# lfilipozzi/PathPlanning

Measured on AMD Instinct MI355X. Metric: hybrid_astar_plans_per_sec_1024x1024, higher is better.
Workload: dtype f64

## Files before the change

__graft_entry__.py:

```python
import os
import subprocess
import sys

os.environ.setdefault("GPU_MAX_HW_QUEUES", "2")

ROOT = os.path.dirname(os.path.abspath(__file__))
if ROOT not in sys.path:
    sys.path.insert(0, ROOT)


def build():
    from pathplanning_amd import build as b
    lib = b.build(force=False)
    assert os.path.exists(lib), lib
    b.build_pyplanning()
    b.build_plugin_test()
    b.build_pipeline_footprint_test()
    b.build_pipeline_postprocess_test()
    b.build_row_test()
    subprocess.check_call(["make", "-C", os.path.join(ROOT, "oracle"), os.path.join(ROOT, "oracle", "libppo.so")])
    if os.path.isdir("/root/reference/planner/src"):
        subprocess.check_call(["make", "-C", os.path.join(ROOT, "oracle"), "ref"])
    subprocess.check_call([sys.executable, "-c", "import ctypes, sys; ctypes.CDLL(sys.argv[1])", lib])
    import pathplanning_amd
    print("built", lib)


def smoke():
    sys.path.insert(0, os.path.join(ROOT, "tests"))
    import numpy as np
    import pathplanning_amd as pa
    import torch
    assert torch.cuda.is_available(), "smoke() needs a GPU"
    import oracle_lib as O
# ... 72 lines not shown
```

pathplanning_amd/build.py:

```python
import os
import subprocess
import sys

HERE = os.path.dirname(os.path.abspath(__file__))
CSRC = os.path.join(HERE, "csrc")
LIB_DIR = os.path.join(HERE, "lib")
LIB = os.path.join(LIB_DIR, "libpphip.so")
SOURCES = ["pp_capi.hip", "pp_kernels_basic.hip", "pp_paths.hip", "pp_footprint.hip", "pp_gvd.hip", "pp_wavefront.hip", "pp_wavefront_tiles.hip", "pp_planner.hip", "pp_rrt.hip", "pp_grid_astar.hip"]
HEADERS = sorted(f for f in os.listdir(CSRC) if f.endswith(".hpp")) + [os.path.join("..", "..", "include", "pp_hip.h")]
FLAGS = ["--offload-arch=gfx950", "-O3", "-std=c++17", "-ffp-contract=off", "-fPIC", "-shared"]


def hipcc():
    for c in (os.environ.get("HIPCC"), "/opt/rocm/bin/hipcc", "hipcc"):
        if c and (os.path.isabs(c) and os.path.exists(c) or not os.path.isabs(c)):
            return c
    return "hipcc"


def stale():
    if not os.path.exists(LIB):
        return True
    t = os.path.getmtime(LIB)
    deps = [os.path.join(CSRC, s) for s in SOURCES + HEADERS]
# ... 63 lines not shown
    return out


def build_row_test(verbose=True):
    out = os.path.join(LIB_DIR, "test_row_primitives")
    src = os.path.join(HERE, "..", "tests", "cpp", "test_row_primitives.hip")
    if os.path.exists(out) and os.path.getmtime(out) > max(os.path.getmtime(src), os.path.getmtime(os.path.join(CSRC, "pp_row_primitives.hpp"))):
        return out
    cmd = [hipcc(), "--offload-arch=gfx950", "-O2", "-I", CSRC, "-I", os.path.join(HERE, "..", "include"), src, "-o", out]
    if verbose:
        print(" ".join(cmd), file=sys.stderr)
    subprocess.check_call(cmd)
    return out


if __name__ == "__main__":
    build(force="--force" in sys.argv)
    print(LIB)
    print(build_pyplanning())
    print(build_plugin_test())
    print(build_pipeline_footprint_test())
    print(build_pipeline_postprocess_test())
    print(build_row_test())
```

pathplanning_amd/csrc/pp_capi.hip:

```cpp
#include "pp_internal.hpp"

#include <cmath>
#include <cstdio>
#include <cstring>
#include <memory>

namespace pph {

static thread_local std::string g_lastError;

void set_error(const std::string& msg) { g_lastError = msg; }
int hip_fail(hipError_t e, const char* what)
{
	g_lastError = std::string(what) + ": " + hipGetErrorString(e);
	return e == hipErrorNoDevice ? PP_ERR_NO_DEVICE : PP_ERR_HIP;
}

}

using namespace pph;

ppd::MapView pp_map::view() const
{
	ppd::MapView v;
// ... 445 lines not shown
		return PP_ERR_INVALID;
	}
	if (!map->pathcost) {
		set_error("path-cost grid not uploaded (pp_map_upload_path_cost)");
		return PP_ERR_INVALID;
	}
	rp.arcLength = params->spatial_resolution * 1.5;
	rp.spatialRes = params->spatial_resolution;
	rp.angularRes = params->angular_resolution;
	rp.lat.set(params->spatial_resolution, params->angular_resolution);
	rp.forwardMult = params->forward_cost_multiplier;
	rp.reverseMult = params->reverse_cost_multiplier;
	rp.voronoiMult = params->voronoi_cost_multiplier;
	rp.voroDiagRes = (float)(map->desc.resolution * std::sqrt(2.0));
	rp.headingAlias = params->heading_alias;
	pt.n = n_primitives;
	for (int i = 0; i < n_primitives; i++) {
		pt.kappa[i] = curvature_host[i];
		pt.invKappa[i] = curvature_host[i] != 0.0 ? 1 / curvature_host[i] : 0.0;
		pt.backward[i] = direction_host[i] == 1;
	}
	return PP_OK;
}

int pp_rollout_children_dev(pp_map* map, const pp_hybrid_params* params, int32_t n_primitives, const double* curvature_host, const int32_t* direction_host,
	int64_t n_parents, const double* parents_dev, uint8_t* valid_dev, double* pose_dev, int32_t* key_dev, double* cost_dev, double* length_dev)
{
	if (int rc = check_map(map, true))
		return rc;
	RolloutParams rp;
// ... 467 lines not shown
```

pathplanning_amd/csrc/pp_device.hpp:

```cpp
#pragma once

#include <hip/hip_runtime.h>
#include <stdint.h>

namespace ppd {

#define PPD_INLINE __device__ __forceinline__

constexpr double kPi = 3.14159265358979323846;

#ifndef PP_FIELD_TILE_LOG2
#define PP_FIELD_TILE_LOG2 3
#endif
constexpr int kFieldTileLog2 = PP_FIELD_TILE_LOG2, kFieldTile = 1 << kFieldTileLog2, kFieldTileMask = kFieldTile - 1;
__host__ __device__ inline size_t field_tiled_index(int cols, int row, int col)
{
	const int tpr = (cols + kFieldTileMask) >> kFieldTileLog2;
	return ((size_t)((row >> kFieldTileLog2) * tpr + (col >> kFieldTileLog2)) << (2 * kFieldTileLog2)) | (size_t)(((row & kFieldTileMask) << kFieldTileLog2) | (col & kFieldTileMask));
}
__host__ __device__ inline size_t field_tiled_elems(int rows, int cols)
{
	return (size_t)((rows + kFieldTileMask) >> kFieldTileLog2) * (size_t)((cols + kFieldTileMask) >> kFieldTileLog2) * (size_t)(kFieldTile * kFieldTile);
}
constexpr double kPi2 = 1.57079632679489661923;
// ... 131 lines not shown
		lt = wrap_theta(theta);
	const double qx = div_by(x - m.gx, (double)m.res, m.invRes), qy = div_by(y - m.gy, (double)m.res, m.invRes);
	const bool inRange = qx > -2147483649.0 && qx < 2147483648.0 && qy > -2147483649.0 && qy < 2147483648.0;
	const int row = (int)qx, col = (int)qy;
	const bool bounds = !(lx < m.lbx) & !(lx > m.ubx) & !(ly < m.lby) & !(ly > m.uby) & !(lt < m.lbt) & !(lt > m.ubt);
	const bool inside = inRange & ((unsigned)row < (unsigned)m.rows) & ((unsigned)col < (unsigned)m.cols);
#ifdef PP_CS_EXPERIMENT_NO_GATHER
	const uint32_t cell = inside ? (uint32_t)(row & 1) : 0u;
#else
	const uint32_t cell = inside ? (uint32_t)row * (uint32_t)m.cols + (uint32_t)col : 0u;
#endif
	const uint32_t bit = (validBits[cell >> 5] >> (cell & 31)) & 1u;
	return bounds & inside & (bit != 0u);
}

PPD_INLINE Pose constant_steer(const Pose& from, double kappa, double dist)
{
	Pose to = from;
	if (fabs(kappa) > 1e-9) {
		to.t += dist * kappa;
		to.x += 1 / kappa * (sin(to.t) - sin(from.t));
		to.y += 1 / kappa * (-cos(to.t) + cos(from.t));
	} else {
		to.x += dist * cos(from.t);
		to.y += dist * sin(from.t);
	}
	return to;
}

struct Arc {
// ... 31 lines not shown
			to.t += d * kappa;
			sincos(to.t, &s, &c);
			to.x += invKappa * (s - sinF);
			to.y += invKappa * (-c + cosF);
		} else {
			to.x += d * cosF;
			to.y += d * sinF;
		}
		return to;
	}
	PPD_INLINE Pose interpolate(double ratio) const
	{
		double s, c;
		return interpolate_sc(ratio, s, c);
	}
};

struct Segment {
	double x0, y0, x1, y1;
	double length;
	PPD_INLINE Pose interpolate(double ratio) const
	{
		Pose p;
		p.x = (1 - ratio) * x0 + ratio * x1;
		p.y = (1 - ratio) * y0 + ratio * y1;
		p.t = 0.0;
		return p;
	}
};

PPD_INLINE float fmin4(double a, double b, double c, double d)
// ... 29 lines not shown
		checks++;
		if (!is_state_valid(m, s.x, s.y, s.t, distance)) {
			last = (float)(lastValidLength / pathLength);
			return false;
		}
		lastValidLength = length;
		float distToMapBorder = fmin4(s.x - m.lbx, m.ubx - s.x, s.y - m.lby, m.uby - s.y);
		float deltaLength = distance - m.minSafeRadius;
		deltaLength = fminf(deltaLength, distToMapBorder);
		length += (double)fmaxf(deltaLength, m.minInterp);
	}
	last = 1.0f;
	return true;
}

template <typename PathT>
PPD_INLINE bool is_path_valid_from(const MapView& m, const PathT& path, const Pose& init, float firstDist, float& last, int& checks)
{
	const double pathLength = path.length;
	if (pathLength == 0.0) {
		last = 1.0f;
		checks++;
		return !(firstDist < 0.0f);
	}
	checks++;
	if (firstDist < 0.0f) {
		last = 0.0f;
		return false;
	}
	float distance = firstDist;
	double lastValidLength = 0.0;
	double length = 0.0;
	{
		const float distToMapBorder = fmin4(init.x - m.lbx, m.ubx - init.x, init.y - m.lby, m.uby - init.y);
		float deltaLength = distance - m.minSafeRadius;
		deltaLength = fminf(deltaLength, distToMapBorder);
		length += (double)fmaxf(deltaLength, m.minInterp);
	}
	while (length < pathLength) {
		if (checks > (1 << 22)) {
			last = (float)(lastValidLength / pathLength);
			return false;
		}
		Pose s = path.interpolate(length / pathLength);
		checks++;
		if (!is_state_valid(m, s.x, s.y, s.t, distance)) {
			last = (float)(lastValidLength / pathLength);
			return false;
		}
		lastValidLength = length;
		float distToMapBorder = fmin4(s.x - m.lbx, m.ubx - s.x, s.y - m.lby, m.uby - s.y);
		float deltaLength = distance - m.minSafeRadius;
		deltaLength = fminf(deltaLength, distToMapBorder);
		length += (double)fmaxf(deltaLength, m.minInterp);
	}
	last = 1.0f;
	return true;
}

template <typename PathT>
PPD_INLINE double voronoi_cost(const MapView& m, const PathT& path, float interpLength, double voronoiCostMultiplier)
{
	float voronoiCost = 0.0f;
	const double pathLength = path.length;
	if (0.0 < pathLength) {
		double lastLength = 0.0;
		if (interpLength > 0.0f)
			for (double length = 0.0; length < pathLength; length += (double)interpLength) {
				if (length == lastLength && length != 0.0)
					break;
				lastLength = length;
			}
		Pose p = path.interpolate(lastLength / pathLength);
		int row, col;
		world_to_cell(m, p.x, p.y, row, col);
		row = min(max(row, 0), m.rows - 1);
		col = min(max(col, 0), m.cols - 1);
		voronoiCost = m.pathcost[(size_t)row * m.cols + col];
	}
	voronoiCost *= interpLength;
	return voronoiCostMultiplier * (double)voronoiCost;
}

template <typename PathT>
PPD_INLINE void voronoi_cost_issue(const MapView& m, const PathT& path, float interpLength, float& raw)
{
	raw = 0.0f;
	const double pathLength = path.length;
	if (0.0 < pathLength) {
		double lastLength = 0.0;
		if (interpLength > 0.0f)
			for (double length = 0.0; length < pathLength; length += (double)interpLength) {
				if (length == lastLength && length != 0.0)
					break;
				lastLength = length;
			}
		Pose p = path.interpolate(lastLength / pathLength);
		int row, col;
		world_to_cell(m, p.x, p.y, row, col);
		row = min(max(row, 0), m.rows - 1);
		col = min(max(col, 0), m.cols - 1);
		raw = m.pathcost[(size_t)row * m.cols + col];
	}
}
PPD_INLINE double voronoi_cost_finish(float raw, float interpLength, double voronoiCostMultiplier)
{
	float voronoiCost = raw;
	voronoiCost *= interpLength;
	return voronoiCostMultiplier * (double)voronoiCost;
}

PPD_INLINE int alias_heading_bin(int theta)
{
	int t = theta;
	while ((double)t > kPi)
		t = (int)((double)t - 2 * kPi);
	while ((double)t < -kPi)
		t = (int)((double)t + 2 * kPi);
// ... 20 lines not shown
```

pathplanning_amd/csrc/pp_footprint_device.hpp:

```cpp
#pragma once

#include "pp_device.hpp"

namespace ppd {

constexpr int kFootprintMaxDiscs = 8;

struct Footprint {
	int n;
	int anyOffset;
	double rho;
	double ox[kFootprintMaxDiscs], oy[kFootprintMaxDiscs];
	float r[kFootprintMaxDiscs];
	int slot[kFootprintMaxDiscs];
};

PPD_INLINE void disc_centre(const Footprint& fp, int i, double x, double y, double s, double c, double& cx, double& cy)
{
	if (fp.ox[i] == 0.0 && fp.oy[i] == 0.0) {
		cx = x;
		cy = y;
	} else {
		cx = (x + fp.ox[i] * c) - fp.oy[i] * s;
		cy = (y + fp.ox[i] * s) + fp.oy[i] * c;
// ... 154 lines not shown
	last = 1.0f;
	return true;
}

PPD_INLINE float fp_border_sc(const MapView& m, const Footprint& fp, double x, double y, double s, double c)
{
	double b = dmin4(x - m.lbx, m.ubx - x, y - m.lby, m.uby - y, __builtin_huge_val());
	for (int i = 0; i < fp.n; i++) {
		double cx, cy;
		disc_centre(fp, i, x, y, s, c, cx, cy);
		b = dmin4(b, cx - m.lbx, m.ubx - cx, cy - m.lby, m.uby - cy);
	}
	return (float)b;
}

PPD_INLINE bool is_arc_valid_fp_from(const MapView& m, const Footprint& fp, float gain, const ArcSC& path, float firstClearance, float& last, int& checks)
{
	const double pathLength = path.length;
	if (pathLength == 0.0) {
		last = 1.0f;
		checks++;
		return !(firstClearance < 0.0f);
	}
	checks++;
	if (firstClearance < 0.0f) {
		last = 0.0f;
		return false;
	}
	double lastValidLength = 0.0;
	double length = 0.0;
	{
		const float border = fp_border_sc(m, fp, path.init.x, path.init.y, path.sinF, path.cosF);
		const float deltaLength = fminf(firstClearance, border) / gain;
		length += (double)fmaxf(deltaLength, m.minInterp);
	}
	while (length < pathLength) {
		if (checks > (1 << 22)) {
			last = (float)(lastValidLength / pathLength);
			return false;
		}
		double s, c;
		const Pose p = path.interpolate_sc(length / pathLength, s, c);
		checks++;
		float clearance, border;
		if (!fp_state_valid_sc(m, fp, p.x, p.y, p.t, s, c, clearance, border)) {
			last = (float)(lastValidLength / pathLength);
			return false;
		}
		lastValidLength = length;
		const float deltaLength = fminf(clearance, border) / gain;
		length += (double)fmaxf(deltaLength, m.minInterp);
	}
	last = 1.0f;
	return true;
}

}
```

pathplanning_amd/csrc/pp_internal.hpp:

```cpp
#pragma once

#include <hip/hip_runtime.h>
#include <stdint.h>
#include <string>
#include <vector>

#include "../../include/pp_hip.h"
#include "pp_device.hpp"
#include "pp_footprint_device.hpp"

namespace pph {

void set_error(const std::string& msg);
int hip_fail(hipError_t e, const char* what);

#define PP_HIP_TRY(expr)                       \
	do {                                       \
		hipError_t _e = (expr);                \
		if (_e != hipSuccess)                  \
			return pph::hip_fail(_e, #expr);   \
	} while (0)

template <typename H, hipError_t (*Release)(H)>
class Owner {
// ... 51 lines not shown
constexpr int kMaxPrimitives = 128;
struct PrimTable {
	int n;
	double kappa[kMaxPrimitives];
	double invKappa[kMaxPrimitives];
	int8_t backward[kMaxPrimitives];
};

struct RolloutParams {
	double arcLength;
	double spatialRes, angularRes;
	ppd::Resolutions lat;
	double forwardMult, reverseMult, voronoiMult;
	float voroDiagRes;
	int headingAlias;
};

struct NonHoloDesc {
	int nx, ny, na;
	double spatialRes, angularRes, offX, offY;
	double rmin;
	float reverseCost, forwardCost, switchCost;
	double minMult;
	int negativeKRead;
};

hipError_t launch_d2_to_distance(hipStream_t s, const int32_t* d2, float* dist, int64_t n, float res);
hipError_t launch_occ_to_u8(hipStream_t s, const int32_t* occ, uint8_t* occ8, int64_t n);
hipError_t launch_check_states(hipStream_t s, const ppd::MapView& m, int64_t n, const double* poses, uint8_t* valid);
hipError_t launch_check_states_fused(hipStream_t s, const ppd::MapView& m, int64_t n, uint64_t seed, uint64_t* count);
// ... 147 lines not shown
```

pathplanning_amd/csrc/pp_kernels_basic.hip:

```cpp
#include "pp_internal.hpp"

#include <mutex>

#include <cstdlib>
#include "pp_rs_device.hpp"

using namespace ppd;

namespace {

constexpr int kBlock = 256;

inline int grid_for(int64_t n, int block, int maxBlocks = 256 * 16)
{
	int64_t b = (n + block - 1) / block;
	if (b < 1)
		b = 1;
	if (b > maxBlocks)
		b = maxBlocks;
	return (int)b;
}

__global__ void k_d2_to_distance(const int32_t* __restrict__ d2, float* __restrict__ dist, int64_t n, float res)
{
// ... 227 lines not shown
		discretize_pose(child, rp.lat, rp.headingAlias, ix, iy, it);
		float lastValidRatio;
		int checks = 0;
		bool ok = true;
		if (!is_path_valid(m, a, a.init, lastValidRatio, checks)) {
			child = a.interpolate((double)lastValidRatio);
			a.length *= (double)lastValidRatio;
			discretize_pose(child, rp.lat, rp.headingAlias, ix, iy, it);
			if (ix == pix && iy == piy && it == pit)
				ok = false;
		}
		double c = 0.0;
		if (ok) {
			double pathCost = (a.backward ? rp.reverseMult : rp.forwardMult) * a.length;
			double switchingCost = 0.0;
			double voro = voronoi_cost(m, a, rp.voroDiagRes, rp.voronoiMult);
			c = pathCost + switchingCost + voro;
		}
		valid[idx] = ok ? 1 : 0;
		pose[3 * idx] = child.x;
		pose[3 * idx + 1] = child.y;
		pose[3 * idx + 2] = child.t;
		key[3 * idx] = ix;
		key[3 * idx + 1] = iy;
		key[3 * idx + 2] = it;
		cost[idx] = c;
		lengthOut[idx] = ok ? a.length : 0.0;
	}
}

__global__ void __launch_bounds__(kBlock) k_rs_solve(int64_t n, const double* __restrict__ from, const double* __restrict__ to, double rmin, float rev, float fwd,
// ... 225 lines not shown
```

pathplanning_amd/csrc/pp_planner.hip:

```cpp
#include "pp_search_device.hpp"
#include "pp_row_primitives.hpp"

#include <cmath>
#include <cstring>
#include <memory>
#include <string>
#include <utility>
#include <vector>

using namespace ppd;

namespace {

struct Node {
	double x, y, t;
	double pathCost, totalCost;
	double length;
	double h;
	double sinT, cosT;
	int32_t parent;
	uint32_t key;
	int16_t action;
	uint8_t dead;
	uint8_t pad0;
// ... 456 lines not shown
	SearchArgs& A = p->args;
	A.m = map->view();
	if (int rc = primitives_from_deltas(p)) {
		free_planner(p);
		return rc;
	}
	A.rp.arcLength = params->spatial_resolution * 1.5;
	A.rp.spatialRes = params->spatial_resolution;
	A.rp.angularRes = params->angular_resolution;
	A.rp.lat.set(params->spatial_resolution, params->angular_resolution);
	A.rp.forwardMult = params->forward_cost_multiplier;
	A.rp.reverseMult = params->reverse_cost_multiplier;
	A.rp.voronoiMult = params->voronoi_cost_multiplier;
	A.rp.voroDiagRes = (float)(map->desc.resolution * std::sqrt(2.0));
	A.rp.headingAlias = params->heading_alias;
	int32_t dims[3];
	double offs[2];
	if (int rc = pp_nonholo_dims(map->desc.lower, map->desc.upper, params, dims, offs)) {
		free_planner(p);
		return rc;
	}
	A.heur.nx = dims[0];
	A.heur.ny = dims[1];
	A.heur.na = dims[2];
	A.heur.spatialRes = params->spatial_resolution;
	A.heur.angularRes = params->angular_resolution;
	A.heur.lat.set(params->spatial_resolution, params->angular_resolution);
	A.heur.offX = offs[0];
	A.heur.offY = offs[1];
	A.heur.minMult = std::min(params->reverse_cost_multiplier, params->forward_cost_multiplier);
// ... 814 lines not shown
```

pathplanning_amd/csrc/pp_planner_rows.hpp:

```cpp
#ifndef PP_ROWS_FOOTPRINT
#error "pp_planner_rows.hpp is the body of the rows kernels of pp_planner.hip, which defines PP_ROWS_FOOTPRINT before each include"
#endif

#ifndef PP_ROWS_PREAMBLE_DONE
#define PP_ROWS_PREAMBLE_DONE 1
#ifndef PP_ROWS_STATS
#define PP_ROWS_STATS 0
#endif
#if PP_ROWS_STATS
__device__ unsigned long long g_rowsStats[24];
#endif
#ifndef PP_ROWS_WAVES_PER_WG
#define PP_ROWS_WAVES_PER_WG 4
#endif
#if PP_ROWS_STATS
#undef PP_ROWS_WAVES_PER_WG
#define PP_ROWS_WAVES_PER_WG 1
#endif
#ifndef PP_ROWS_EAGER_REFILL
#define PP_ROWS_EAGER_REFILL 1
#endif

#ifndef PP_PIPE_POLL_EVERY
#define PP_PIPE_POLL_EVERY 8
// ... 62 lines not shown
	};
	static_assert(offsetof(WaveLds, bandCnt) % 16 == 0 && sizeof(WaveLds) % 16 == 0, "band counters are copied as uint4");
	__shared__ __attribute__((aligned(16))) WaveLds s_wave[kW];
	WaveLds& W = s_wave[threadIdx.x >> 6];
	double *const c_x = W.c_x, *const c_y = W.c_y, *const c_t = W.c_t, *const c_cost = W.c_cost, *const c_total = W.c_total, *const c_len = W.c_len, *const c_h = W.c_h,
		   *const c_sin = W.c_sin, *const c_cos = W.c_cos, *const f_x = W.f_x, *const f_y = W.f_y, *const f_t = W.f_t, *const f_tot = W.f_tot;
	uint32_t *const c_key = W.c_key, *const c_state = W.c_state, *const f_for = W.f_for;
	float* const c_d0 = W.c_d0;
	uint8_t *const c_flags = W.c_flags, *const c_valid = W.c_valid;
	int16_t* const c_action = W.c_action;
	int* const s_rsChecks = W.rsChecks;
	HeapEntry* const spillBuf = W.spill[lane >> 4];
	uint32_t* const bandCnt = W.bandCnt[lane >> 4];

	const MapView& m = A.m;
	const int P = A.prims.n;
	const int maxNodes = A.maxNodes;

	int q = -1;
	bool act = false, done = false;
	const float* field = nullptr;
	Pose goal = { 0, 0, 0 };
	int myNode = -1, rsNode = -1;
	int pfNode = -1;
	unsigned long long pf64 = 0ull;
	bool pfDead = false;
	FrontLane front;
	front_clear(front);
	int frontCount = 0, heapSize = 0, nSpill = 0;
	int nOutside = 0;
// ... 529 lines not shown
			bool ok = false;
			uint32_t key = kNoKey, st = 0u;
			Pose child = ppose;
			double cs = pSin, cc = pCos;
			double gcost = 0.0, total = 0.0, len = 0.0, hh = 0.0;
			float d0 = -1.0f;
			if (p < P) {
				ArcSC a;
				a.init = ppose;
				a.sinF = pSin;
				a.cosF = pCos;
				a.kappa = A.prims.kappa[p];
				a.invKappa = A.prims.invKappa[p];
				a.length = A.rp.arcLength;
				a.backward = A.prims.backward[p];
				child = a.interpolate_sc(1.0, cs, cc);
				int ix, iy, it;
				lanePathChecks += (long long)discretize_pose(child, A.rp.lat, A.rp.headingAlias, ix, iy, it) << kGuardShift;
				ROWS_STAMP(11)
				bool packed = A.ks.pack(ix, iy, it, key);
				if (packed)
					st = keymap[key];
				HeurLoads hl;
				combined_heuristic_issue(A.heur, m, field, goal, child, cs, cc, hl);
				ROWS_STAMP(12)
				float voroRaw;
				voronoi_cost_issue(m, a, A.rp.voroDiagRes, voroRaw);
				ROWS_STAMP(13)
				float lastValidRatio;
				int checks = 0;
				ok = true;
				lanePathChecks++;
				float cd0;
#if PP_ROWS_FOOTPRINT
				float cRaw[kFootprintMaxDiscs];
				const bool cIn = fp_state_valid_issue_sc(m, foot, child.x, child.y, child.t, cs, cc, cRaw);
#else
				const bool cIn = is_state_valid_issue(m, child.x, child.y, child.t, cd0);
#endif
				ROWS_STAMP(4)
#if PP_ROWS_FOOTPRINT
				const bool pathValid = is_arc_valid_fp_from(m, foot, fp_gain(foot, fabs(a.kappa)), a, pDist0, lastValidRatio, checks);
#else
				const bool pathValid = is_path_valid_from(m, a, a.init, pDist0, lastValidRatio, checks);
#endif
				ROWS_STAMP(5)
				hh = combined_heuristic_finish(A.heur, hl);
				const double voroFull = voronoi_cost_finish(voroRaw, A.rp.voroDiagRes, A.rp.voronoiMult);
#if PP_ROWS_FOOTPRINT
				d0 = fp_state_valid_finish(foot, cIn, cRaw, cd0) ? cd0 : -1.0f;
#else
				d0 = is_state_valid_finish(m, cIn, cd0) ? cd0 : -1.0f;
#endif
				if (!pathValid) {
					child = a.interpolate_sc((double)lastValidRatio, cs, cc);
					a.length *= (double)lastValidRatio;
					lanePathChecks += (long long)discretize_pose(child, A.rp.lat, A.rp.headingAlias, ix, iy, it) << kGuardShift;
					if (ix == pix && iy == piy && it == pit)
						ok = false;
					else {
						packed = A.ks.pack(ix, iy, it, key);
						if (packed)
							st = keymap[key];
						hh = combined_heuristic_sc(A.heur, m, field, goal, child, cs, cc);
#if PP_ROWS_FOOTPRINT
						float cb;
						d0 = fp_state_valid_sc(m, foot, child.x, child.y, child.t, cs, cc, cd0, cb) ? cd0 : -1.0f;
#else
						d0 = is_state_valid(m, child.x, child.y, child.t, cd0) ? cd0 : -1.0f;
#endif
					}
				}
				laneStateChecks += checks;
				if (ok) {
					const double pathCost = (a.backward ? A.rp.reverseMult : A.rp.forwardMult) * a.length;
					const double voro = pathValid ? voroFull : voronoi_cost(m, a, A.rp.voroDiagRes, A.rp.voronoiMult);
					const double cost = pathCost + 0.0 + voro;
					len = a.length;
					gcost = pPathCost + cost;
					total = gcost + hh;
					if (!packed)
						ok = false;
				}
			}
			ROWS_STAMP(6)
			if (ok && key == pKey)
				st = kExplored;
			double fpx = 0.0, fpy = 0.0, fpt = 0.0, fptot = 0.0;
			uint32_t fpFor = 0u;
			wave_vmem_sync();
			if (ok && st != 0u && st != kExplored) {
// ... 203 lines not shown
					double* const pre = W.rsPre[lane >> 4];
					path.make_prefix(pre);
					const rs::PrefixedPath ppath = { path, pre, path.length };
#if PP_ROWS_FOOTPRINT
					const bool valid = is_path_valid_fp(m, foot, fp_gain(foot, 1.0 / A.rmin), ppath, path.init, lastRatio, checks);
#else
					const bool valid = is_path_valid(m, ppath, path.init, lastRatio, checks);
#endif
					c_valid[sb + kRowRs] = 0;
					s_rsChecks[lane >> 4] = checks;
					if (valid) {
						const double pathAndSwitchingCosts = (double)rs::compute_cost(path.seg, A.rmin, A.rsRev, A.rsFwd, A.rsSw);
						const Pose child = ppath.interpolate(1.0);
						int ix, iy, it;
						lanePathChecks += (long long)discretize_pose(child, A.rp.lat, A.rp.headingAlias, ix, iy, it) << kGuardShift;
						const double voro = voronoi_cost(m, ppath, A.rp.voroDiagRes, A.rp.voronoiMult);
						const double cost = pathAndSwitchingCosts + voro;
						uint32_t key;
						if (A.ks.pack(ix, iy, it, key)) {
							double s_, c_;
							sincos(child.t, &s_, &c_);
							const double hh = combined_heuristic_sc(A.heur, m, field, goal, child, s_, c_);
							c_valid[sb + kRowRs] = 1;
							c_key[sb + kRowRs] = key;
							c_x[sb + kRowRs] = child.x;
							c_y[sb + kRowRs] = child.y;
							c_t[sb + kRowRs] = child.t;
							c_cost[sb + kRowRs] = pPathCost + cost;
							c_total[sb + kRowRs] = (pPathCost + cost) + hh;
							c_len[sb + kRowRs] = path.length;
							c_h[sb + kRowRs] = hh;
// ... 118 lines not shown
```

pathplanning_amd/csrc/pp_search_body.hpp:

```cpp
#ifndef PP_SEARCH_BODY_INCLUDER
#error "pp_search_body.hpp is the body of the search kernels of pp_planner.hip; it is not a header to include elsewhere"
#endif
	if (resume ? ((int)blockIdx.x >= *nResume || (int)blockIdx.x >= A.listCap) : (int)blockIdx.x >= nQueries)
		return;
	const SuspendRec rec = resume ? resume[blockIdx.x] : SuspendRec {};
	const int q = resume ? rec.q : (int)blockIdx.x;
	const size_t slot = resume ? (size_t)rec.slot : (size_t)q;
	const int lane = threadIdx.x;
#if PP_SEARCH_SETPRIO
	__builtin_amdgcn_s_setprio(3);
#endif
	unsigned long long phase[PH_COUNT] = { 0, 0, 0, 0, 0, 0, 0, 0 };
	unsigned long long tlast = 0;
	if (kProfile)
		tlast = clock64();
#define PP_STAMP(i)                                \
	if (kProfile) {                                \
		const unsigned long long now_ = clock64(); \
		phase[i] += now_ - tlast;                  \
		tlast = now_;                              \
	}

	__shared__ unsigned long long mt[Mt64::N];
	__shared__ double c_x[kSlots], c_y[kSlots], c_t[kSlots], c_cost[kSlots], c_total[kSlots], c_len[kSlots], c_h[kSlots], c_sin[kSlots], c_cos[kSlots];
	__shared__ uint32_t c_key[kSlots], c_state[kSlots];
	__shared__ float c_d0[kSlots];
	__shared__ uint8_t c_valid[kSlots];
	__shared__ int16_t c_action[kSlots];
	__shared__ int s_rsChecks;
	__shared__ double s_rsPre[24];
	__shared__ HeapEntry s_spill[16];
	__shared__ uint8_t s_bandCnt[kBands];

	const MapView& m = A.m;
	const int P = A.prims.n;
	const int maxNodes = A.maxNodes;
	Node* nodes = nodesBase + slot * maxNodes;
	HeapEntry* heap = heapBase + slot * maxNodes;
	HeapEntry* bands = bandBase + slot * (size_t)(kBands * kBandCap);
	uint32_t* keymap = keymapBase + slot * A.ks.size();
	uint32_t* expanded = expandedBase + (size_t)q * maxNodes;
	RsLogEntry* rsLog = rsLogBase + (size_t)q * kRsLogCap;
	const float* field = costFields + (size_t)q * A.fieldElems;

	const Pose start = { starts[3 * q], starts[3 * q + 1], wrap_theta(starts[3 * q + 2]) };
	const Pose goal = { goals[3 * q], goals[3 * q + 1], wrap_theta(goals[3 * q + 2]) };

	if (!resume) {
		const size_t n = A.ks.size();
// ... 318 lines not shown
				a.length = A.rp.arcLength;
				a.backward = A.prims.backward[p];
				child = a.interpolate_sc(1.0, cs, cc);
				int ix, iy, it;
				const bool onLine = discretize_pose(child, A.rp.lat, A.rp.headingAlias, ix, iy, it);
				lanePathChecks += (long long)onLine << kGuardShift;
				if (onLine)
					guard_log(A, q, ni, p, 1, a.length, ix, iy, it);
				PP_STAMP(PH_HEUR);
				bool packed = A.ks.pack(ix, iy, it, key);
				if (packed)
					st = keymap[key];
				HeurLoads hl;
				combined_heuristic_issue(A.heur, m, field, goal, child, cs, cc, hl);
				float voroRaw;
				voronoi_cost_issue(m, a, A.rp.voroDiagRes, voroRaw);
				float lastValidRatio;
				int checks = 0;
				ok = true;
				lanePathChecks++;
				float cd0;
				bool cIn, pathValid;
				if constexpr (kFootprint) {
					cIn = false;
					pathValid = is_arc_valid_fp_from(m, foot, fp_gain(foot, fabs(a.kappa)), a, pDist0, lastValidRatio, checks);
				} else {
					cIn = is_state_valid_issue(m, child.x, child.y, child.t, cd0);
					pathValid = is_path_valid_from(m, a, a.init, pDist0, lastValidRatio, checks);
				}
				PP_STAMP(PH_DUP);
				hh = combined_heuristic_finish(A.heur, hl);
				const double voroFull = voronoi_cost_finish(voroRaw, A.rp.voroDiagRes, A.rp.voronoiMult);
				if constexpr (kFootprint) {
					float cb;
					d0 = pathValid && fp_state_valid_sc(m, foot, child.x, child.y, child.t, cs, cc, cd0, cb) ? cd0 : -1.0f;
				} else
					d0 = is_state_valid_finish(m, cIn, cd0) ? cd0 : -1.0f;
				if (!pathValid) {
					child = a.interpolate_sc((double)lastValidRatio, cs, cc);
					a.length *= (double)lastValidRatio;
					const bool onLineT = discretize_pose(child, A.rp.lat, A.rp.headingAlias, ix, iy, it);
					lanePathChecks += (long long)onLineT << kGuardShift;
					if (onLineT)
// ... 3 lines not shown
					else {
						packed = A.ks.pack(ix, iy, it, key);
						if (packed)
							st = keymap[key];
						hh = combined_heuristic_sc(A.heur, m, field, goal, child, cs, cc);
						if constexpr (kFootprint) {
							float cb;
							d0 = fp_state_valid_sc(m, foot, child.x, child.y, child.t, cs, cc, cd0, cb) ? cd0 : -1.0f;
						} else
							d0 = is_state_valid(m, child.x, child.y, child.t, cd0) ? cd0 : -1.0f;
					}
				}
				laneStateChecks += checks;
				if (ok) {
					const double pathCost = (a.backward ? A.rp.reverseMult : A.rp.forwardMult) * a.length;
					const double voro = pathValid ? voroFull : voronoi_cost(m, a, A.rp.voroDiagRes, A.rp.voronoiMult);
					const double cost = pathCost + 0.0 + voro;
					len = a.length;
					gcost = pPathCost + cost;
					total = gcost + hh;
					if (!packed)
						ok = false;
				}
			}
			if (ok && key == pKey)
				st = kExplored;
			double fpx = 0.0, fpy = 0.0, fpt = 0.0, fptot = 0.0;
			uint32_t fpFor = 0u;
			wave_vmem_sync();
			if (ok && st != 0u && st != kExplored) {
				const Node* fn = nodes + (st - 1u);
// ... 193 lines not shown
					bool valid;
					if constexpr (kFootprint)
						valid = is_path_valid_fp(m, foot, fp_gain(foot, 1.0 / A.rmin), ppath, path.init, lastRatio, checks);
					else
						valid = is_path_valid(m, ppath, path.init, lastRatio, checks);
					c_valid[kRsSlot] = 0;
					s_rsChecks = checks;
					if (valid) {
						const double pathAndSwitchingCosts = (double)rs::compute_cost(path.seg, A.rmin, A.rsRev, A.rsFwd, A.rsSw);
						const Pose child = ppath.interpolate(1.0);
						int ix, iy, it;
						const bool onLineR = discretize_pose(child, A.rp.lat, A.rp.headingAlias, ix, iy, it);
						lanePathChecks += (long long)onLineR << kGuardShift;
						if (onLineR)
							guard_log(A, q, ni, word, 2, path.length, ix, iy, it);
						const double voro = voronoi_cost(m, ppath, A.rp.voroDiagRes, A.rp.voronoiMult);
						const double cost = pathAndSwitchingCosts + voro;
						uint32_t key;
						if (A.ks.pack(ix, iy, it, key)) {
							double s_, c_;
							sincos(child.t, &s_, &c_);
							const double hh = combined_heuristic_sc(A.heur, m, field, goal, child, s_, c_);
							c_valid[kRsSlot] = 1;
							c_key[kRsSlot] = key;
							c_x[kRsSlot] = child.x;
							c_y[kRsSlot] = child.y;
							c_t[kRsSlot] = child.t;
							c_cost[kRsSlot] = pPathCost + cost;
							c_total[kRsSlot] = (pPathCost + cost) + hh;
							c_len[kRsSlot] = path.length;
							c_h[kRsSlot] = hh;
// ... 131 lines not shown
```

Baseline: 36550.

## Precompute full-arc voronoi ratio, batch sincos, and overlap truncated-arc loads

Precomputes on the host the voronoi sample ratio and reciprocal arc length for the fixed full primitive length, which avoids the per-child sampling loop and division. Computes the child pose and the voronoi sample pose from one shared heading evaluation using a custom wave-uniform fast sincos with a fallback for large arguments. In the rows kernel the truncated-arc path now issues heuristic, state and voronoi loads before finishing them, to overlap memory latency. This adds bit-exactness risk in the custom sincos and in the reciprocal-multiply division.

```diff
diff --git a/__graft_entry__.py b/__graft_entry__.py
--- a/__graft_entry__.py
+++ b/__graft_entry__.py
@@ -18,6 +18,7 @@
     b.build_pipeline_footprint_test()
     b.build_pipeline_postprocess_test()
     b.build_row_test()
+    b.build_sincos_test()
     subprocess.check_call(["make", "-C", os.path.join(ROOT, "oracle"), os.path.join(ROOT, "oracle", "libppo.so")])
     if os.path.isdir("/root/reference/planner/src"):
         subprocess.check_call(["make", "-C", os.path.join(ROOT, "oracle"), "ref"])
diff --git a/pathplanning_amd/build.py b/pathplanning_amd/build.py
--- a/pathplanning_amd/build.py
+++ b/pathplanning_amd/build.py
@@ -101,6 +101,19 @@
     return out
 
 
+def build_sincos_test(verbose=True):
+    out = os.path.join(LIB_DIR, "test_sincos_multi")
+    src = os.path.join(HERE, "..", "tests", "cpp", "test_sincos_multi.hip")
+    if os.path.exists(out) and os.path.getmtime(out) > max(os.path.getmtime(src), os.path.getmtime(os.path.join(CSRC, "pp_device.hpp"))):
+        return out
+    os.makedirs(LIB_DIR, exist_ok=True)
+    cmd = [hipcc()] + [f for f in FLAGS if f not in ("-fPIC", "-shared")] + ["-I", CSRC, src, "-o", out]
+    if verbose:
+        print(" ".join(cmd), file=sys.stderr)
+    subprocess.check_call(cmd)
+    return out
+
+
 if __name__ == "__main__":
     build(force="--force" in sys.argv)
     print(LIB)
@@ -109,3 +122,4 @@
     print(build_pipeline_footprint_test())
     print(build_pipeline_postprocess_test())
     print(build_row_test())
+    print(build_sincos_test())
diff --git a/pathplanning_amd/csrc/pp_arc_host.hpp b/pathplanning_amd/csrc/pp_arc_host.hpp
--- /dev/null
+++ b/pathplanning_amd/csrc/pp_arc_host.hpp
@@ -0,0 +1,38 @@
+#pragma once
+
+namespace pph {
+
+struct ArcConstants {
+	double voroLastLength;
+	double voroLastRatio;
+	double invArcLength;
+	int arcDivBy;
+};
+
+inline void voronoi_last_sample(double pathLength, float interpLength, double& lastLength, double& lastRatio)
+{
+	lastLength = 0.0;
+	lastRatio = 0.0;
+	if (!(0.0 < pathLength))
+		return;
+	if (interpLength > 0.0f)
+		for (double length = 0.0; length < pathLength; length += (double)interpLength) {
+			if (length == lastLength && length != 0.0)
+				break;
+			lastLength = length;
+		}
+	lastRatio = lastLength / pathLength;
+}
+
+inline bool div_by_holds(double b) { return b >= 0x1p-400 && b <= 0x1p400; }
+
+inline ArcConstants arc_constants(double arcLength, float voroDiagRes)
+{
+	ArcConstants c;
+	voronoi_last_sample(arcLength, voroDiagRes, c.voroLastLength, c.voroLastRatio);
+	c.arcDivBy = div_by_holds(arcLength) ? 1 : 0;
+	c.invArcLength = c.arcDivBy ? 1.0 / arcLength : 0.0;
+	return c;
+}
+
+}
diff --git a/pathplanning_amd/csrc/pp_capi.hip b/pathplanning_amd/csrc/pp_capi.hip
--- a/pathplanning_amd/csrc/pp_capi.hip
+++ b/pathplanning_amd/csrc/pp_capi.hip
@@ -483,6 +483,7 @@
 	rp.voronoiMult = params->voronoi_cost_multiplier;
 	rp.voroDiagRes = (float)(map->desc.resolution * std::sqrt(2.0));
 	rp.headingAlias = params->heading_alias;
+	rp.finish_arc();
 	pt.n = n_primitives;
 	for (int i = 0; i < n_primitives; i++) {
 		pt.kappa[i] = curvature_host[i];
diff --git a/pathplanning_amd/csrc/pp_device.hpp b/pathplanning_amd/csrc/pp_device.hpp
--- a/pathplanning_amd/csrc/pp_device.hpp
+++ b/pathplanning_amd/csrc/pp_device.hpp
@@ -169,6 +169,85 @@
 	return bounds & inside & (bit != 0u);
 }
 
+constexpr double kSincosSmallBound = 1073741824.0;
+constexpr double f64_bits(unsigned long long b) { return __builtin_bit_cast(double, b); }
+
+PPD_INLINE void sincos_small(double x, double& sinOut, double& cosOut)
+{
+	const double ax = fabs(x);
+	const double n = rint(ax * f64_bits(0x3FE45F306DC9C883ull));
+	const double r0 = __builtin_fma(n, f64_bits(0xBFF921FB54442D18ull), ax);
+	const double r1 = __builtin_fma(n, f64_bits(0xBC91A62633145C00ull), r0);
+	const double pl = n * f64_bits(0x3C91A62633145C00ull);
+	const double pe = __builtin_fma(n, f64_bits(0x3C91A62633145C00ull), -pl);
+	const double t0 = r0 - pl;
+	const double t1 = r0 - t0;
+	const double t2 = t1 - pl;
+	const double t3 = t0 - r1;
+	const double t4 = t3 + t2;
+	const double t5 = t4 - pe;
+	const double t6 = __builtin_fma(n, f64_bits(0xB97B839A252049C0ull), t5);
+	const double hi = r1 + t6;
+	const double t7 = hi - r1;
+	const double lo = t6 - t7;
+	const int q = (int)n & 3;
+	const double z = hi * hi;
+	const double hz = z * 0.5;
+	const double c1 = 1.0 - hz;
+	const double c2 = 1.0 - c1;
+	const double c3 = c2 - hz;
+	const double zz = z * z;
+	double cp = __builtin_fma(z, f64_bits(0xBDA907DB46CC5E42ull), f64_bits(0x3E21EEB69037AB78ull));
+	cp = __builtin_fma(z, cp, f64_bits(0xBE927E4FA17F65F6ull));
+	cp = __builtin_fma(z, cp, f64_bits(0x3EFA01A019F4EC90ull));
+	cp = __builtin_fma(z, cp, f64_bits(0xBF56C16C16C16967ull));
+	cp = __builtin_fma(z, cp, f64_bits(0x3FA5555555555555ull));
+	const double nlo = -lo;
+	const double c4 = __builtin_fma(hi, nlo, c3);
+	const double c5 = __builtin_fma(zz, cp, c4);
+	const double cr = c1 + c5;
+	double sp = __builtin_fma(z, f64_bits(0x3DE5E0B2F9A43BB8ull), f64_bits(0xBE5AE600B42FDFA7ull));
+	sp = __builtin_fma(z, sp, f64_bits(0x3EC71DE3796CDE01ull));
+	sp = __builtin_fma(z, sp, f64_bits(0xBF2A01A019E83E5Cull));
+	sp = __builtin_fma(z, sp, f64_bits(0x3F81111111110BB3ull));
+	const double nz3 = hi * -z;
+	const double hl = lo * 0.5;
+	const double s1 = __builtin_fma(nz3, sp, hl);
+	const double s2 = __builtin_fma(z, s1, nlo);
+	const double s3 = __builtin_fma(nz3, f64_bits(0xBFC5555555555555ull), s2);
+	const double sr = hi - s3;
+	const unsigned long long flip = q > 1 ? 0x8000000000000000ull : 0ull;
+	const bool even = (q & 1) == 0;
+	const unsigned long long sb = (unsigned long long)__double_as_longlong(even ? sr : cr);
+	const unsigned long long cb = (unsigned long long)__double_as_longlong(even ? cr : -sr);
+	sinOut = __longlong_as_double((long long)(sb ^ ((unsigned long long)__double_as_longlong(x) & 0x8000000000000000ull) ^ flip));
+	cosOut = __longlong_as_double((long long)(cb ^ flip));
+}
+PPD_INLINE bool sincos_is_small(double x) { return fabs(x) < kSincosSmallBound; }
+
+PPD_INLINE void sincos2(double a, double b, double& sa, double& ca, double& sb, double& cb)
+{
+	if (__ballot(!(sincos_is_small(a) && sincos_is_small(b))) != 0ull) {
+		sincos(a, &sa, &ca);
+		sincos(b, &sb, &cb);
+		return;
+	}
+	sincos_small(a, sa, ca);
+	sincos_small(b, sb, cb);
+}
+PPD_INLINE void sincos3(double a, double b, double c, double& sa, double& ca, double& sb, double& cb, double& sc, double& cc)
+{
+	if (__ballot(!(sincos_is_small(a) && sincos_is_small(b) && sincos_is_small(c))) != 0ull) {
+		sincos(a, &sa, &ca);
+		sincos(b, &sb, &cb);
+		sincos(c, &sc, &cc);
+		return;
+	}
+	sincos_small(a, sa, ca);
+	sincos_small(b, sb, cb);
+	sincos_small(c, sc, cc);
+}
+
 PPD_INLINE Pose constant_steer(const Pose& from, double kappa, double dist)
 {
 	Pose to = from;
@@ -230,7 +309,57 @@
 		double s, c;
 		return interpolate_sc(ratio, s, c);
 	}
-};
+	PPD_INLINE double travel(double ratio) const
+	{
+		const double d = length * ratio;
+		return backward ? -d : d;
+	}
+	PPD_INLINE double heading_at(double d) const { return init.t + d * kappa; }
+	PPD_INLINE Pose pose_at(double d, double t, double st, double ct, double& s, double& c) const
+	{
+		Pose to = init;
+		s = sinF;
+		c = cosF;
+		if (d == 0.0)
+			return to;
+		if (fabs(kappa) > 1e-9) {
+			to.t = t;
+			s = st;
+			c = ct;
+			to.x += invKappa * (s - sinF);
+			to.y += invKappa * (-c + cosF);
+		} else {
+			to.x += d * cosF;
+			to.y += d * sinF;
+		}
+		return to;
+	}
+	PPD_INLINE void interpolate2_sc(double r1, double r2, Pose& p1, double& s1, double& c1, Pose& p2, double& s2, double& c2) const
+	{
+		const double d1 = travel(r1), d2 = travel(r2);
+		const double t1 = heading_at(d1), t2 = heading_at(d2);
+		double st1, ct1, st2, ct2;
+		sincos2(t1, t2, st1, ct1, st2, ct2);
+		p1 = pose_at(d1, t1, st1, ct1, s1, c1);
+		p2 = pose_at(d2, t2, st2, ct2, s2, c2);
+	}
+};
+
+struct FullArc {
+	double length;
+	double voroLastRatio;
+	double invLength;
+	int divBy;
+};
+
+PPD_INLINE FullArc no_full_arc() { return FullArc{ __builtin_nan(""), 0.0, 0.0, 0 }; }
+
+PPD_INLINE double length_ratio(double len, double pathLength, const FullArc& fa)
+{
+	if (fa.divBy && pathLength == fa.length)
+		return div_by(len, pathLength, fa.invLength);
+	return len / pathLength;
+}
 
 struct Segment {
 	double x0, y0, x1, y1;
@@ -290,8 +419,16 @@
 	return true;
 }
 
+PPD_INLINE double march_first_length(const MapView& m, const Pose& init, float firstDist)
+{
+	const float distToMapBorder = fmin4(init.x - m.lbx, m.ubx - init.x, init.y - m.lby, m.uby - init.y);
+	float deltaLength = firstDist - m.minSafeRadius;
+	deltaLength = fminf(deltaLength, distToMapBorder);
+	return 0.0 + (double)fmaxf(deltaLength, m.minInterp);
+}
+
 template <typename PathT>
-PPD_INLINE bool is_path_valid_from(const MapView& m, const PathT& path, const Pose& init, float firstDist, float& last, int& checks)
+PPD_INLINE bool is_path_valid_from(const MapView& m, const PathT& path, const Pose& init, float firstDist, const FullArc& fa, float& last, int& checks)
 {
 	const double pathLength = path.length;
 	if (pathLength == 0.0) {
@@ -306,22 +443,16 @@
 	}
 	float distance = firstDist;
 	double lastValidLength = 0.0;
-	double length = 0.0;
-	{
-		const float distToMapBorder = fmin4(init.x - m.lbx, m.ubx - init.x, init.y - m.lby, m.uby - init.y);
-		float deltaLength = distance - m.minSafeRadius;
-		deltaLength = fminf(deltaLength, distToMapBorder);
-		length += (double)fmaxf(deltaLength, m.minInterp);
-	}
+	double length = march_first_length(m, init, firstDist);
 	while (length < pathLength) {
 		if (checks > (1 << 22)) {
-			last = (float)(lastValidLength / pathLength);
+			last = (float)length_ratio(lastValidLength, pathLength, fa);
 			return false;
 		}
-		Pose s = path.interpolate(length / pathLength);
+		Pose s = path.interpolate(length_ratio(length, pathLength, fa));
 		checks++;
 		if (!is_state_valid(m, s.x, s.y, s.t, distance)) {
-			last = (float)(lastValidLength / pathLength);
+			last = (float)length_ratio(lastValidLength, pathLength, fa);
 			return false;
 		}
 		lastValidLength = length;
@@ -334,50 +465,46 @@
 	return true;
 }
 
+PPD_INLINE double voronoi_sample_ratio(double pathLength, float interpLength, const FullArc& fa)
+{
+	if (pathLength == fa.length)
+		return fa.voroLastRatio;
+	double lastLength = 0.0;
+	if (interpLength > 0.0f)
+		for (double length = 0.0; length < pathLength; length += (double)interpLength) {
+			if (length == lastLength && length != 0.0)
+				break;
+			lastLength = length;
+		}
+	return lastLength / pathLength;
+}
+PPD_INLINE float voronoi_read(const MapView& m, const Pose& p)
+{
+	int row, col;
+	world_to_cell(m, p.x, p.y, row, col);
+	row = min(max(row, 0), m.rows - 1);
+	col = min(max(col, 0), m.cols - 1);
+	return m.pathcost[(size_t)row * m.cols + col];
+}
+
 template <typename PathT>
-PPD_INLINE double voronoi_cost(const MapView& m, const PathT& path, float interpLength, double voronoiCostMultiplier)
+PPD_INLINE double voronoi_cost(const MapView& m, const PathT& path, float interpLength, double voronoiCostMultiplier, const FullArc& fa)
 {
 	float voronoiCost = 0.0f;
 	const double pathLength = path.length;
-	if (0.0 < pathLength) {
-		double lastLength = 0.0;
-		if (interpLength > 0.0f)
-			for (double length = 0.0; length < pathLength; length += (double)interpLength) {
-				if (length == lastLength && length != 0.0)
-					break;
-				lastLength = length;
-			}
-		Pose p = path.interpolate(lastLength / pathLength);
-		int row, col;
-		world_to_cell(m, p.x, p.y, row, col);
-		row = min(max(row, 0), m.rows - 1);
-		col = min(max(col, 0), m.cols - 1);
-		voronoiCost = m.pathcost[(size_t)row * m.cols + col];
-	}
+	if (0.0 < pathLength)
+		voronoiCost = voronoi_read(m, path.interpolate(voronoi_sample_ratio(pathLength, interpLength, fa)));
 	voronoiCost *= interpLength;
 	return voronoiCostMultiplier * (double)voronoiCost;
 }
 
 template <typename PathT>
-PPD_INLINE void voronoi_cost_issue(const MapView& m, const PathT& path, float interpLength, float& raw)
+PPD_INLINE void voronoi_cost_issue(const MapView& m, const PathT& path, float interpLength, const FullArc& fa, float& raw)
 {
 	raw = 0.0f;
 	const double pathLength = path.length;
-	if (0.0 < pathLength) {
-		double lastLength = 0.0;
-		if (interpLength > 0.0f)
-			for (double length = 0.0; length < pathLength; length += (double)interpLength) {
-				if (length == lastLength && length != 0.0)
-					break;
-				lastLength = length;
-			}
-		Pose p = path.interpolate(lastLength / pathLength);
-		int row, col;
-		world_to_cell(m, p.x, p.y, row, col);
-		row = min(max(row, 0), m.rows - 1);
-		col = min(max(col, 0), m.cols - 1);
-		raw = m.pathcost[(size_t)row * m.cols + col];
-	}
+	if (0.0 < pathLength)
+		raw = voronoi_read(m, path.interpolate(voronoi_sample_ratio(pathLength, interpLength, fa)));
 }
 PPD_INLINE double voronoi_cost_finish(float raw, float interpLength, double voronoiCostMultiplier)
 {
diff --git a/pathplanning_amd/csrc/pp_footprint_device.hpp b/pathplanning_amd/csrc/pp_footprint_device.hpp
--- a/pathplanning_amd/csrc/pp_footprint_device.hpp
+++ b/pathplanning_amd/csrc/pp_footprint_device.hpp
@@ -192,7 +192,7 @@
 	return (float)b;
 }
 
-PPD_INLINE bool is_arc_valid_fp_from(const MapView& m, const Footprint& fp, float gain, const ArcSC& path, float firstClearance, float& last, int& checks)
+PPD_INLINE bool is_arc_valid_fp_from(const MapView& m, const Footprint& fp, float gain, const ArcSC& path, float firstClearance, const FullArc& fa, float& last, int& checks)
 {
 	const double pathLength = path.length;
 	if (pathLength == 0.0) {
@@ -214,15 +214,15 @@
 	}
 	while (length < pathLength) {
 		if (checks > (1 << 22)) {
-			last = (float)(lastValidLength / pathLength);
+			last = (float)length_ratio(lastValidLength, pathLength, fa);
 			return false;
 		}
 		double s, c;
-		const Pose p = path.interpolate_sc(length / pathLength, s, c);
+		const Pose p = path.interpolate_sc(length_ratio(length, pathLength, fa), s, c);
 		checks++;
 		float clearance, border;
 		if (!fp_state_valid_sc(m, fp, p.x, p.y, p.t, s, c, clearance, border)) {
-			last = (float)(lastValidLength / pathLength);
+			last = (float)length_ratio(lastValidLength, pathLength, fa);
 			return false;
 		}
 		lastValidLength = length;
diff --git a/pathplanning_amd/csrc/pp_internal.hpp b/pathplanning_amd/csrc/pp_internal.hpp
--- a/pathplanning_amd/csrc/pp_internal.hpp
+++ b/pathplanning_amd/csrc/pp_internal.hpp
@@ -6,6 +6,7 @@
 #include <vector>
 
 #include "../../include/pp_hip.h"
+#include "pp_arc_host.hpp"
 #include "pp_device.hpp"
 #include "pp_footprint_device.hpp"
 
@@ -89,6 +90,18 @@
 	double forwardMult, reverseMult, voronoiMult;
 	float voroDiagRes;
 	int headingAlias;
+	double voroLastLength, voroLastRatio;
+	double invArcLength;
+	int arcDivBy;
+	void finish_arc()
+	{
+		const ArcConstants c = arc_constants(arcLength, voroDiagRes);
+		voroLastLength = c.voroLastLength;
+		voroLastRatio = c.voroLastRatio;
+		invArcLength = c.invArcLength;
+		arcDivBy = c.arcDivBy;
+	}
+	__host__ __device__ ppd::FullArc full_arc() const { return ppd::FullArc{ arcLength, voroLastRatio, invArcLength, arcDivBy }; }
 };
 
 struct NonHoloDesc {
diff --git a/pathplanning_amd/csrc/pp_kernels_basic.hip b/pathplanning_amd/csrc/pp_kernels_basic.hip
--- a/pathplanning_amd/csrc/pp_kernels_basic.hip
+++ b/pathplanning_amd/csrc/pp_kernels_basic.hip
@@ -265,7 +265,7 @@
 		if (ok) {
 			double pathCost = (a.backward ? rp.reverseMult : rp.forwardMult) * a.length;
 			double switchingCost = 0.0;
-			double voro = voronoi_cost(m, a, rp.voroDiagRes, rp.voronoiMult);
+			double voro = voronoi_cost(m, a, rp.voroDiagRes, rp.voronoiMult, rp.full_arc());
 			c = pathCost + switchingCost + voro;
 		}
 		valid[idx] = ok ? 1 : 0;
diff --git a/pathplanning_amd/csrc/pp_planner.hip b/pathplanning_amd/csrc/pp_planner.hip
--- a/pathplanning_amd/csrc/pp_planner.hip
+++ b/pathplanning_amd/csrc/pp_planner.hip
@@ -494,6 +494,7 @@
 	A.rp.voronoiMult = params->voronoi_cost_multiplier;
 	A.rp.voroDiagRes = (float)(map->desc.resolution * std::sqrt(2.0));
 	A.rp.headingAlias = params->heading_alias;
+	A.rp.finish_arc();
 	int32_t dims[3];
 	double offs[2];
 	if (int rc = pp_nonholo_dims(map->desc.lower, map->desc.upper, params, dims, offs)) {
diff --git a/pathplanning_amd/csrc/pp_planner_rows.hpp b/pathplanning_amd/csrc/pp_planner_rows.hpp
--- a/pathplanning_amd/csrc/pp_planner_rows.hpp
+++ b/pathplanning_amd/csrc/pp_planner_rows.hpp
@@ -100,6 +100,7 @@
 	uint32_t* const bandCnt = W.bandCnt[lane >> 4];
 
 	const MapView& m = A.m;
+	const FullArc fullArc = A.rp.full_arc();
 	const int P = A.prims.n;
 	const int maxNodes = A.maxNodes;
 
@@ -659,7 +660,12 @@
 				a.invKappa = A.prims.invKappa[p];
 				a.length = A.rp.arcLength;
 				a.backward = A.prims.backward[p];
-				child = a.interpolate_sc(1.0, cs, cc);
+				const bool voroOn = 0.0 < a.length;
+				const double voroRatio = voroOn ? voronoi_sample_ratio(a.length, A.rp.voroDiagRes, fullArc) : 0.0;
+				Pose voroPose;
+				double vs, vc;
+				a.interpolate2_sc(1.0, voroRatio, child, cs, cc, voroPose, vs, vc);
+				const float voroRaw = voroOn ? voronoi_read(m, voroPose) : 0.0f;
 				int ix, iy, it;
 				lanePathChecks += (long long)discretize_pose(child, A.rp.lat, A.rp.headingAlias, ix, iy, it) << kGuardShift;
 				ROWS_STAMP(11)
@@ -669,8 +675,6 @@
 				HeurLoads hl;
 				combined_heuristic_issue(A.heur, m, field, goal, child, cs, cc, hl);
 				ROWS_STAMP(12)
-				float voroRaw;
-				voronoi_cost_issue(m, a, A.rp.voroDiagRes, voroRaw);
 				ROWS_STAMP(13)
 				float lastValidRatio;
 				int checks = 0;
@@ -679,27 +683,35 @@
 				float cd0;
 #if PP_ROWS_FOOTPRINT
 				float cRaw[kFootprintMaxDiscs];
-				const bool cIn = fp_state_valid_issue_sc(m, foot, child.x, child.y, child.t, cs, cc, cRaw);
+				bool cIn = fp_state_valid_issue_sc(m, foot, child.x, child.y, child.t, cs, cc, cRaw);
 #else
-				const bool cIn = is_state_valid_issue(m, child.x, child.y, child.t, cd0);
+				bool cIn = is_state_valid_issue(m, child.x, child.y, child.t, cd0);
 #endif
 				ROWS_STAMP(4)
 #if PP_ROWS_FOOTPRINT
-				const bool pathValid = is_arc_valid_fp_from(m, foot, fp_gain(foot, fabs(a.kappa)), a, pDist0, lastValidRatio, checks);
+				const bool pathValid = is_arc_valid_fp_from(m, foot, fp_gain(foot, fabs(a.kappa)), a, pDist0, fullArc, lastValidRatio, checks);
 #else
-				const bool pathValid = is_path_valid_from(m, a, a.init, pDist0, lastValidRatio, checks);
+				const bool pathValid = is_path_valid_from(m, a, a.init, pDist0, fullArc, lastValidRatio, checks);
 #endif
 				ROWS_STAMP(5)
 				hh = combined_heuristic_finish(A.heur, hl);
-				const double voroFull = voronoi_cost_finish(voroRaw, A.rp.voroDiagRes, A.rp.voronoiMult);
+				double voro = voronoi_cost_finish(voroRaw, A.rp.voroDiagRes, A.rp.voronoiMult);
 #if PP_ROWS_FOOTPRINT
 				d0 = fp_state_valid_finish(foot, cIn, cRaw, cd0) ? cd0 : -1.0f;
 #else
 				d0 = is_state_valid_finish(m, cIn, cd0) ? cd0 : -1.0f;
 #endif
 				if (!pathValid) {
-					child = a.interpolate_sc((double)lastValidRatio, cs, cc);
-					a.length *= (double)lastValidRatio;
+					const double truncRatio = (double)lastValidRatio;
+					const double dEnd = a.travel(truncRatio);
+					a.length *= truncRatio;
+					const bool tvOn = 0.0 < a.length;
+					const double dVoro = tvOn ? a.travel(voronoi_sample_ratio(a.length, A.rp.voroDiagRes, no_full_arc())) : 0.0;
+					const double tEnd = a.heading_at(dEnd), tVoro = a.heading_at(dVoro);
+					double se, ce, sv, cv;
+					sincos2(tEnd, tVoro, se, ce, sv, cv);
+					child = a.pose_at(dEnd, tEnd, se, ce, cs, cc);
+					voroPose = a.pose_at(dVoro, tVoro, sv, cv, vs, vc);
 					lanePathChecks += (long long)discretize_pose(child, A.rp.lat, A.rp.headingAlias, ix, iy, it) << kGuardShift;
 					if (ix == pix && iy == piy && it == pit)
 						ok = false;
@@ -707,19 +719,25 @@
 						packed = A.ks.pack(ix, iy, it, key);
 						if (packed)
 							st = keymap[key];
-						hh = combined_heuristic_sc(A.heur, m, field, goal, child, cs, cc);
+						combined_heuristic_issue(A.heur, m, field, goal, child, cs, cc, hl);
 #if PP_ROWS_FOOTPRINT
-						float cb;
-						d0 = fp_state_valid_sc(m, foot, child.x, child.y, child.t, cs, cc, cd0, cb) ? cd0 : -1.0f;
+						cIn = fp_state_valid_issue_sc(m, foot, child.x, child.y, child.t, cs, cc, cRaw);
 #else
-						d0 = is_state_valid(m, child.x, child.y, child.t, cd0) ? cd0 : -1.0f;
-#endif
+						cIn = is_state_valid_issue(m, child.x, child.y, child.t, cd0);
+#endif
+						const float tvRaw = tvOn ? voronoi_read(m, voroPose) : 0.0f;
+						hh = combined_heuristic_finish(A.heur, hl);
+#if PP_ROWS_FOOTPRINT
+						d0 = fp_state_valid_finish(foot, cIn, cRaw, cd0) ? cd0 : -1.0f;
+#else
+						d0 = is_state_valid_finish(m, cIn, cd0) ? cd0 : -1.0f;
+#endif
+						voro = voronoi_cost_finish(tvRaw, A.rp.voroDiagRes, A.rp.voronoiMult);
 					}
 				}
 				laneStateChecks += checks;
 				if (ok) {
 					const double pathCost = (a.backward ? A.rp.reverseMult : A.rp.forwardMult) * a.length;
-					const double voro = pathValid ? voroFull : voronoi_cost(m, a, A.rp.voroDiagRes, A.rp.voronoiMult);
 					const double cost = pathCost + 0.0 + voro;
 					len = a.length;
 					gcost = pPathCost + cost;
@@ -953,7 +971,7 @@
 						const Pose child = ppath.interpolate(1.0);
 						int ix, iy, it;
 						lanePathChecks += (long long)discretize_pose(child, A.rp.lat, A.rp.headingAlias, ix, iy, it) << kGuardShift;
-						const double voro = voronoi_cost(m, ppath, A.rp.voroDiagRes, A.rp.voronoiMult);
+						const double voro = voronoi_cost(m, ppath, A.rp.voroDiagRes, A.rp.voronoiMult, no_full_arc());
 						const double cost = pathAndSwitchingCosts + voro;
 						uint32_t key;
 						if (A.ks.pack(ix, iy, it, key)) {
diff --git a/pathplanning_amd/csrc/pp_search_body.hpp b/pathplanning_amd/csrc/pp_search_body.hpp
--- a/pathplanning_amd/csrc/pp_search_body.hpp
+++ b/pathplanning_amd/csrc/pp_search_body.hpp
@@ -33,6 +33,7 @@
 	__shared__ uint8_t s_bandCnt[kBands];
 
 	const MapView& m = A.m;
+	const FullArc fullArc = A.rp.full_arc();
 	const int P = A.prims.n;
 	const int maxNodes = A.maxNodes;
 	Node* nodes = nodesBase + slot * maxNodes;
@@ -381,7 +382,7 @@
 				HeurLoads hl;
 				combined_heuristic_issue(A.heur, m, field, goal, child, cs, cc, hl);
 				float voroRaw;
-				voronoi_cost_issue(m, a, A.rp.voroDiagRes, voroRaw);
+				voronoi_cost_issue(m, a, A.rp.voroDiagRes, fullArc, voroRaw);
 				float lastValidRatio;
 				int checks = 0;
 				ok = true;
@@ -390,10 +391,10 @@
 				bool cIn, pathValid;
 				if constexpr (kFootprint) {
 					cIn = false;
-					pathValid = is_arc_valid_fp_from(m, foot, fp_gain(foot, fabs(a.kappa)), a, pDist0, lastValidRatio, checks);
+					pathValid = is_arc_valid_fp_from(m, foot, fp_gain(foot, fabs(a.kappa)), a, pDist0, fullArc, lastValidRatio, checks);
 				} else {
 					cIn = is_state_valid_issue(m, child.x, child.y, child.t, cd0);
-					pathValid = is_path_valid_from(m, a, a.init, pDist0, lastValidRatio, checks);
+					pathValid = is_path_valid_from(m, a, a.init, pDist0, fullArc, lastValidRatio, checks);
 				}
 				PP_STAMP(PH_DUP);
 				hh = combined_heuristic_finish(A.heur, hl);
@@ -427,7 +428,7 @@
 				laneStateChecks += checks;
 				if (ok) {
 					const double pathCost = (a.backward ? A.rp.reverseMult : A.rp.forwardMult) * a.length;
-					const double voro = pathValid ? voroFull : voronoi_cost(m, a, A.rp.voroDiagRes, A.rp.voronoiMult);
+					const double voro = pathValid ? voroFull : voronoi_cost(m, a, A.rp.voroDiagRes, A.rp.voronoiMult, fullArc);
 					const double cost = pathCost + 0.0 + voro;
 					len = a.length;
 					gcost = pPathCost + cost;
@@ -651,7 +652,7 @@
 						lanePathChecks += (long long)onLineR << kGuardShift;
 						if (onLineR)
 							guard_log(A, q, ni, word, 2, path.length, ix, iy, it);
-						const double voro = voronoi_cost(m, ppath, A.rp.voroDiagRes, A.rp.voronoiMult);
+						const double voro = voronoi_cost(m, ppath, A.rp.voroDiagRes, A.rp.voronoiMult, fullArc);
 						const double cost = pathAndSwitchingCosts + voro;
 						uint32_t key;
 						if (A.ks.pack(ix, iy, it, key)) {
```

Result: faster. 37690 (median of 6 runs) (+3.1%).
